# chjj/lcdb

Hardware: AMD Instinct MI355X
Metric: device-resident GiB/s Snappy encode+decode, 4 KiB blocks, 1/2/4/8 MI355X (higher is better)
Workload: dtype u8

## Files before the change

### lcdb_amd/csrc/lgs_api.cpp

```cpp

#include <hip/hip_runtime.h>

#include <stdarg.h>
#include <stdint.h>
#include <stdio.h>
#include <stdlib.h>
#include <string.h>
#include <unistd.h>

#include <atomic>
#include <chrono>
#include <condition_variable>
#include <deque>
#include <functional>
#include <memory>
#include <mutex>
#include <thread>
#include <unordered_map>
#include <vector>

#include "../../include/lcdb_gpu_snappy.h"

#include "lgs_block.h"
#include "lgs_launch.h"
// ... 748 lines not shown
      svc_stage(c, xp, n);
      uint32_t st = 0, olen = 0;
      const int rc = svc_call(*sv, c, 1, n, &st, &olen);
      if (rc == LGS_OK) {
        if (st == LGS_ST_OK && olen != want)
          return fail(LGS_EINTERNAL, "service decode: %u bytes for a %u-byte header", olen, want);
        if (st == LGS_ST_OK) memcpy(zp, h + kSvcOut, want);
        *ok = st == LGS_ST_OK;
        return LGS_OK;
      }
      if (rc != kSvcWithdrawn) return rc;
    }
  }

  Layout L;
  const size_t o_in = L.take((size_t)n + 16);
  const size_t o_ioff = L.take(8);
  const size_t o_ilen = L.take(4);
  const size_t o_ooff = L.take(8);
  const size_t o_ocap = L.take(4);
  const size_t up_end = L.at;
  const size_t o_st = L.take(4);
  const size_t o_olen = L.take(4);
  const size_t o_out = L.take((size_t)want + 16);
  const size_t down_end = L.at;
  if (down_end <= c.h_cap && want <= kInSlotDecodeMax) {
    uint8_t* const hd = c.h_dev;
    (void)up_end;
    memcpy(h + o_in, xp, n);
    memset(h + o_in + n, 0, 16);
    *(uint64_t*)(h + o_ioff) = o_in;
    *(uint32_t*)(h + o_ilen) = n;
    *(uint64_t*)(h + o_ooff) = o_out;
    *(uint32_t*)(h + o_ocap) = want;
    DecodeArgs a{hd, (const uint64_t*)(hd + o_ioff), (const uint32_t*)(hd + o_ilen), hd,
                 (const uint64_t*)(hd + o_ooff), (const uint32_t*)(hd + o_ocap),
                 (uint32_t*)(hd + o_olen), hd + o_st, nullptr, 1, nullptr};
    a.one = Item1{o_in, o_out, n, want, 1};
    LGS_HIP(launch_decode(a, want, c.stream));
    LGS_HIP(hipStreamSynchronize(c.stream));
    const uint8_t st = h[o_st];
    if (st == LGS_ST_OK) memcpy(zp, h + o_out, want);
    *ok = st == LGS_ST_OK;
    return LGS_OK;
  }
  std::unique_ptr<Scratch> guard;
  const size_t big_bytes = align_up((size_t)n + 16, 256) + align_up((size_t)want + 16, 256);
  LGS_TRY(big_alloc(&guard, big_bytes, want, c.stream));
  uint8_t* const big = (uint8_t*)guard->get();
  uint8_t* const d_in = big;
  uint8_t* const d_out = big + align_up((size_t)n + 16, 256);
  Layout M;
  const size_t m_ioff = M.take(8), m_ilen = M.take(4), m_ooff = M.take(8), m_ocap = M.take(4);
  const size_t m_up = M.at;
  const size_t m_st = M.take(4), m_olen = M.take(4);
  const size_t m_down = M.at;
  uint8_t* const d = c.d_buf;
  *(uint64_t*)(h + m_ioff) = 0;
  *(uint32_t*)(h + m_ilen) = n;
  *(uint64_t*)(h + m_ooff) = 0;
  *(uint32_t*)(h + m_ocap) = want;
  LGS_HIP(hipMemcpyAsync(d_in, xp, n, hipMemcpyHostToDevice, c.stream));
  LGS_HIP(hipMemsetAsync(d_in + n, 0, 16, c.stream));
  LGS_HIP(hipMemcpyAsync(d, h, m_up, hipMemcpyHostToDevice, c.stream));
  DecodeArgs a{d_in, (const uint64_t*)(d + m_ioff), (const uint32_t*)(d + m_ilen), d_out,
               (const uint64_t*)(d + m_ooff), (const uint32_t*)(d + m_ocap),
               (uint32_t*)(d + m_olen), d + m_st, nullptr, 1, nullptr};
  LGS_HIP(launch_decode(a, want, c.stream));
  LGS_HIP(hipMemcpyAsync(h + m_st, d + m_st, m_down - m_st, hipMemcpyDeviceToHost, c.stream));
  LGS_HIP(hipStreamSynchronize(c.stream));
  if (h[m_st] == LGS_ST_OK) {
    LGS_HIP(hipMemcpyAsync(zp, d_out, want, hipMemcpyDeviceToHost, c.stream));
    LGS_HIP(hipStreamSynchronize(c.stream));
    *ok = 1;
  }
  return LGS_OK;
}

Options& options_init() {
  static Options* o = [] {
    Options* v = new Options;
    const char* dk = getenv("LGS_DECODE_KERNEL");
    if (dk && !strcmp(dk, "ring")) v->decoder = kDecRing;
    if (dk && !strcmp(dk, "wave")) v->decoder = kDecWave;
#ifdef LGS_PROBE_DECODERS
    if (dk && !strcmp(dk, "chain")) v->decoder = kDecChain;
    if (dk && !strcmp(dk, "group")) v->decoder = kDecGroup;
    const char* wg = getenv("LGS_WIDE_DECODER");
    if (wg && !strcmp(wg, "group")) v->wide = kWideGroup;
    if (dk && !strcmp(dk, "quad")) v->decoder = kDecQuad;
    if (dk && !strcmp(dk, "ops")) v->decoder = kDecOps;
    const char* wd = getenv("LGS_WIDE_DECODER");
    if (wd && !strcmp(wd, "trips")) v->wide = kWideTrips;
#endif
#ifndef LGS_PROBE_DECODERS
    const char* wd0 = getenv("LGS_WIDE_DECODER");
    if ((dk && (!strcmp(dk, "quad") || !strcmp(dk, "ops") || !strcmp(dk, "group") ||
                !strcmp(dk, "chain"))) ||
        (wd0 && (!strcmp(wd0, "trips") || !strcmp(wd0, "group"))))
      fprintf(stderr,
              "lcdb_gpu_snappy: LGS_DECODE_KERNEL=%s LGS_WIDE_DECODER=%s names a probe-library "
              "decoder; this library uses its default decoders\n",
              dk ? dk : "", wd0 ? wd0 : "");
#endif
    const char* vo = getenv("LGS_VERIFY_OVERLAP");
    if (vo && !strcmp(vo, "0")) v->verify_overlap = 0;
    const char* ns = getenv("LGS_NO_SPLIT");
    if (ns && *ns && strcmp(ns, "0")) v->split = 0;
    return v;
  }();
  return *o;
}

}

int set_error(int code, const char* msg) { return fail(code, "%s", msg); }

Options& options() { return options_init(); }

hipError_t launch_fill_stride(uint64_t* off, uint64_t stride, uint32_t n, hipStream_t s);
hipError_t launch_check_lane(const CheckArgs& a, hipStream_t s);

}

using namespace lgs;

extern "C" {


int ldb_snappy_encode_size(size_t* zn, size_t xn) {
  if (xn > 0x7fffffff) return 0;
  const size_t n = bound_of(xn);
  if (n > 0x7fffffff) return 0;
  *zn = n;
  return 1;
}

size_t ldb_snappy_encode(uint8_t* zp, const uint8_t* xp, size_t xn) {
  size_t written = 0;
  if (encode_one(zp, xp, xn, &written) != LGS_OK) die("ldb_snappy_encode");
  return written;
}

int ldb_snappy_decode_size(size_t* zn, const uint8_t* xp, size_t xn) {
  uint32_t v;
  if (!read_varint32(&v, xp, xn)) return 0;
  if (v > 0x7fffffffu) return 0;
  *zn = v;
  return 1;
}

int ldb_snappy_decode(uint8_t* zp, const uint8_t* xp, size_t xn) {
  int ok = 0;
  if (decode_one(zp, xp, xn, &ok) != LGS_OK) die("ldb_snappy_decode");
  return ok;
}


int lgs_dropin_footprint(size_t* pinned, size_t* device, uint32_t* slots, size_t* slot_bytes) {
  if (!pinned || !device || !slots || !slot_bytes) return fail(LGS_EINVAL, "NULL argument");
  unsigned n = 0;
  dropin_pool().footprint(pinned, device, &n);
  *slots = n;
  *slot_bytes = dropin_pool().fixed_cap();
  return LGS_OK;
}

int lgs_service_quiesce(void) { return lgs::svc_quiesce(); }

int lgs_service_resume(void) {
  lgs::g_svc_paused = false;
  return LGS_OK;
}

int lgs_set_option(const char* name, const char* value) {
  if (!name || !value) return fail(LGS_EINVAL, "NULL argument");
  Options& o = options();
  if (!strcmp(name, "decoder")) {
    if (!strcmp(value, "auto") || !*value) o.decoder = kDecAuto;
    else if (!strcmp(value, "ring")) o.decoder = kDecRing;
    else if (!strcmp(value, "wave")) o.decoder = kDecWave;
#ifdef LGS_PROBE_DECODERS
    else if (!strcmp(value, "chain")) o.decoder = kDecChain;
    else if (!strcmp(value, "group")) o.decoder = kDecGroup;
    else if (!strcmp(value, "quad")) o.decoder = kDecQuad;
    else if (!strcmp(value, "ops")) o.decoder = kDecOps;
#endif
    else return fail(LGS_EINVAL, "decoder '%s' (auto, ring or wave)", value);
    return LGS_OK;
  }
  if (!strcmp(name, "inject_alloc_failures")) {
    char* end = nullptr;
    const long v = strtol(value, &end, 10);
    if (!*value || *end || v < 0 || v > 1000000)
      return fail(LGS_EINVAL, "inject_alloc_failures '%s' (0..1000000)", value);
    g_inject_alloc_failures = (int)v;
    return LGS_OK;
  }
  if (!strcmp(name, "wide")) {
    if (!strcmp(value, "walk") || !*value) o.wide = kWideWalk;
#ifdef LGS_PROBE_DECODERS
    else if (!strcmp(value, "group")) o.wide = kWideGroup;
    else if (!strcmp(value, "trips")) o.wide = kWideTrips;
#endif
    else return fail(LGS_EINVAL, "wide '%s' (walk)", value);
    return LGS_OK;
  }
  if (!strcmp(name, "service")) {
    if (!strcmp(value, "1")) g_svc_enabled = 1;
    else if (!strcmp(value, "0")) g_svc_enabled = 0;
    else return fail(LGS_EINVAL, "service '%s' (0 or 1)", value);
    return LGS_OK;
  }
  if (!strcmp(name, "verify_overlap")) {
    if (!strcmp(value, "1")) o.verify_overlap = 1;
    else if (!strcmp(value, "0")) o.verify_overlap = 0;
    else return fail(LGS_EINVAL, "verify_overlap '%s' (0 or 1)", value);
    return LGS_OK;
  }
  if (!strcmp(name, "split")) {
    if (!strcmp(value, "1")) o.split = 1;
    else if (!strcmp(value, "0")) o.split = 0;
    else return fail(LGS_EINVAL, "split '%s' (0 or 1)", value);
    return LGS_OK;
  }
  return fail(LGS_EINVAL, "unknown option '%s'", name);
}


size_t lgs_encode_bound(size_t n) { return bound_of(n); }

int lgs_encode_batch_dev(const uint8_t* d_in, const uint64_t* d_in_off, const uint32_t* d_in_len,
                         uint8_t* d_out, const uint64_t* d_out_off, uint32_t* d_out_len,
                         uint32_t n, uint32_t max_in_len, void* stream) {
  if (n == 0) return LGS_OK;
  if (!d_in || !d_in_off || !d_in_len || !d_out || !d_out_off || !d_out_len)
    return fail(LGS_EINVAL, "NULL argument");
  if (max_in_len > 0x7fffffffu) return fail(LGS_EINVAL, "max_in_len %u too large", max_in_len);
  EncodeArgs a{d_in, d_in_off, d_in_len, d_out, d_out_off, d_out_len, nullptr, nullptr, n, nullptr};
  LGS_HIP(launch_encode(a, max_in_len, (hipStream_t)stream));
  return LGS_OK;
}

int lgs_decode_batch_dev(const uint8_t* d_in, const uint64_t* d_in_off, const uint32_t* d_in_len,
                         uint8_t* d_out, const uint64_t* d_out_off, const uint32_t* d_out_cap,
                         uint32_t* d_out_len, uint8_t* d_status, uint32_t n,
                         uint32_t max_out_cap, void* stream) {
  if (n == 0) return LGS_OK;
  if (!d_in || !d_in_off || !d_in_len || !d_out || !d_out_off || !d_out_cap || !d_out_len ||
      !d_status)
    return fail(LGS_EINVAL, "NULL argument");
  DecodeArgs a{d_in, d_in_off, d_in_len, d_out, d_out_off, d_out_cap, d_out_len, d_status,
               nullptr, n, nullptr};
  LGS_HIP(launch_decode(a, max_out_cap, (hipStream_t)stream));
  return LGS_OK;
}

int lgs_encode_batch_host(const uint8_t* in, const uint64_t* in_off, const uint32_t* in_len,
                          uint8_t* out, const uint64_t* out_off, uint32_t* out_len, uint32_t n) {
  if (n == 0) return LGS_OK;
  if (!in || !in_off || !in_len || !out || !out_off || !out_len)
    return fail(LGS_EINVAL, "NULL argument");
  Lease lease(batch_pool());
// ... 1767 lines not shown
```

### lcdb_amd/csrc/lgs_decode.hip

```cpp
#include "lgs_device.h"
#include "lgs_decode_common.h"
#include "lgs_launch.h"
#include "lgs_probe_hooks.h"
#include "lgs_service.h"

#include <mutex>

namespace lgs {

__device__ uint32_t decode_win(const uint8_t* base, uint32_t sh, uint32_t slen, uint8_t* o,
                               int32_t gap, uint32_t cap, uint32_t* want_out) {
  const uint32_t lane = lane_id();

  const uint64_t w8 = uni64(lds_ld64(base, sh));
  uint32_t want = 0, hlen = 0;
  for (uint32_t i = 0; i < 5 && i < slen; ++i) {
    const uint32_t b = (uint32_t)(w8 >> (8 * i)) & 0xffu;
    if ((b & 0x80u) == 0) {
      want |= b << (7 * i);
      hlen = i + 1;
      break;
    }
    want |= (b & 0x7fu) << (7 * i);
  }
// ... 661 lines not shown
      const uint32_t j = __builtin_amdgcn_mbcnt_hi((uint32_t)(m >> 32),
                                                   __builtin_amdgcn_mbcnt_lo((uint32_t)m, 0));
      const uint32_t total = uni((uint32_t)__builtin_popcountll(m));
      if (need) {
        const uint64_t dp = reinterpret_cast<uint64_t>(dst);
        s_job[j] = RingJob(lane, F, fcnt, dp);
      }
      order();
#pragma clang loop unroll(disable)
      for (uint32_t base = 0; base < total; base += 16) {
        const uint32_t jj = base + (lane >> 2), w = lane & 3u;
        const RingJob jb = s_job[jj];
        if ((jj < total) & (16 * w < jb.cnt)) {
          const uint8_t* rb = s_out + (jb.lane() & (BL - 1)) * kOutStride + 16 +
                              ((uint32_t)jb.ptr() & 15u);
          const u32x4 v0 = lrd16(rb + ((jb.off + 16 * w) & (kOutRing - 1)));
          const bool two = 64 + 16 * w < jb.cnt;
          u32x4 v1 = v0;
          if (two) v1 = lrd16(rb + ((jb.off + 64 + 16 * w) & (kOutRing - 1)));
          const gptr<uint8_t> g = (gptr<uint8_t>)jb.ptr() + jb.off + 16 * w;
          LGS_RING_FLUSH_ST(g, v0, jb.cnt - 16 * w);
          if (two) LGS_RING_FLUSH_ST(g + 64, v1, jb.cnt - 64 - 16 * w);
        }
      }
      order();
      if (need) F += fcnt;
    }
    LGS_RING_PH(3);

    parse(false);
    LGS_RING_PH(4);
    if (TWO) {
      order();
      piece();
      order();
      parse(true);
    }
    LGS_RING_PH(5);

    {
      const uint32_t cons = ((orem > 0) & (okind == 0)) ? olp : pos;
      const bool need = (st == 1) & (in_req < slen) & (in_req <= cons + 64);
      const uint64_t m = ballot(need);
      const uint32_t j = __builtin_amdgcn_mbcnt_hi((uint32_t)(m >> 32),
                                                   __builtin_amdgcn_mbcnt_lo((uint32_t)m, 0));
      const uint32_t total = uni((uint32_t)__builtin_popcountll(m));
      if (need & (j < 32)) {
        const uint64_t sp = reinterpret_cast<uint64_t>(src);
        s_job[j] = RingJob(lane, in_req, slen, sp);
      }
      order();
      ra0 = rm0 = ra1 = rm1 = sink;
      const uint32_t w = lane & 3u;
      if ((lane >> 2) < total) {
        const RingJob jb = s_job[lane >> 2];
        const uint32_t o = jb.off + 16 * w;
        const gptr<const uint8_t> g = (gptr<const uint8_t>)jb.ptr();
        rv0 = ld16(g + (o < jb.cnt ? o : 0u));
        const uint32_t r = o & (kInRing - 1);
        ra0 = jb.lane() * kInStride + r;
        rm0 = r < 64 ? ra0 + kInRing : sink;
      }
      if (16 + (lane >> 2) < total) {
        const RingJob jb = s_job[16 + (lane >> 2)];
        const uint32_t o = jb.off + 16 * w;
        const gptr<const uint8_t> g = (gptr<const uint8_t>)jb.ptr();
        rv1 = ld16(g + (o < jb.cnt ? o : 0u));
        const uint32_t r = o & (kInRing - 1);
        ra1 = jb.lane() * kInStride + r;
        rm1 = r < 64 ? ra1 + kInRing : sink;
      }
      order();
      if (need & (j < 32)) in_req += 64;
    }
    LGS_RING_PH(6);
  } while (ballot(st == 1) & ~(ballot(orem == 0) & ballot(pos >= slen) & ballot(F >= made)));

  if (exists) {
    status[i] = (uint8_t)st;
    out_len[i] = LGS_RING_PH_VALUE(lane, LGS_RING_OUT_LEN(st == 1 ? want : 0));
  }
}

hipError_t launch_decode_ring(const DecodeArgs& a, hipStream_t s) {
#ifndef LGS_RING_BL
#define LGS_RING_BL 32
#endif
  hipLaunchKernelGGL((decode_ring_kernel<true, LGS_RING_BL>), dim3((a.n + LGS_RING_BL - 1) / LGS_RING_BL), dim3(64), 0, s, a.in,
                     a.in_off, a.in_len, a.out, a.out_off, a.out_cap, a.out_len, a.status,
                     a.index, a.n, a.count);
  return hipGetLastError();
}





constexpr uint32_t kDecCap0 = 4608;
constexpr uint32_t kDecCap1 = 16896;
constexpr uint32_t kDecCap2 = 66048;

constexpr uint32_t kLaneMinBlocks = 36864;

__global__ __launch_bounds__(256) void classify_kernel(const uint32_t* __restrict__ len,
                                                       uint32_t n, uint32_t b0, uint32_t b1,
                                                       uint32_t b2, uint32_t* __restrict__ list,
                                                       uint32_t* __restrict__ cnt) {
  const uint32_t i = blockIdx.x * 256 + threadIdx.x;
  const bool here = i < n;
  const uint32_t v = here ? len[i] : 0;
  const uint32_t c = v <= b0 ? 0 : v <= b1 ? 1 : v <= b2 ? 2 : 3;
  const uint32_t lane = lane_id();
  for (uint32_t k = 0; k < 4; ++k) {
    const uint64_t m = __ballot(here && c == k);
    if (m == 0) continue;
    const uint32_t leader = (uint32_t)__ffsll((unsigned long long)m) - 1;
    uint32_t base = 0;
    if (lane == leader) base = atomicAdd(&cnt[k], (uint32_t)__popcll(m));
    base = __shfl(base, leader);
    if (here && c == k) list[(size_t)k * n + base + __popcll(m & ((1ull << lane) - 1))] = i;
  }
}

hipError_t launch_classify(const uint32_t* len, uint32_t n, uint32_t b0, uint32_t b1, uint32_t b2,
                           uint32_t* list, uint32_t* cnt, hipStream_t s) {
  hipLaunchKernelGGL(classify_kernel, dim3((n + 255) / 256), dim3(256), 0, s, len, n, b0, b1, b2,
                     list, cnt);
  return hipGetLastError();
}

static hipMemPool_t scratch_pool(int dev, hipError_t* err) {
  static std::mutex mu;
  static hipMemPool_t pools[64] = {};
  std::lock_guard<std::mutex> g(mu);
  if (dev < 0 || dev >= 64) {
    *err = hipErrorInvalidDevice;
    return nullptr;
  }
  if (!pools[dev]) {
    hipMemPoolProps props = {};
    props.allocType = hipMemAllocationTypePinned;
    props.location.type = hipMemLocationTypeDevice;
    props.location.id = dev;
    hipMemPool_t p = nullptr;
    if ((*err = hipMemPoolCreate(&p, &props)) != hipSuccess) return nullptr;
    uint64_t keep = 256ull << 20;
    (void)hipMemPoolSetAttribute(p, hipMemPoolAttrReleaseThreshold, &keep);
    pools[dev] = p;
  }
  *err = hipSuccess;
  return pools[dev];
}

Scratch::Scratch(size_t bytes, hipStream_t s) : s_(s) {
  int dev = 0;
  err_ = hipGetDevice(&dev);
  if (err_ != hipSuccess) return;
  hipMemPool_t pool = scratch_pool(dev, &err_);
  if (err_ != hipSuccess) return;
  err_ = hipMallocFromPoolAsync(&p_, bytes, pool, s);
  if (err_ != hipSuccess) p_ = nullptr;
}

#define LGS_TRY(x) do { const hipError_t e_ = (x); if (e_ != hipSuccess) return e_; } while (0)

template <uint32_t OUT, uint32_t IN>
static hipError_t launch_decode_wide(const DecodeArgs& a, hipStream_t s) {
  hipLaunchKernelGGL((decode_wide_kernel<OUT, IN>), dim3(a.n), dim3(64), 0, s, a.in, a.in_off,
                     a.in_len, a.out, a.out_off, a.out_cap, a.out_len, a.status, a.index, a.n,
                     a.count);
  return hipGetLastError();
}
static hipError_t launch_decode_big(const DecodeArgs& a, uint32_t max_out, hipStream_t s) {
  (void)max_out;
#ifdef LGS_PROBE_DECODERS
  if (options().wide.load(std::memory_order_relaxed) == kWideTrips)
    return launch_decode_trips(a, s);
#endif
#ifdef LGS_PROBE_DECODERS
  if (max_out <= kGroupMaxOut && (options().wide.load(std::memory_order_relaxed) == kWideGroup ||
                                  options().decoder.load(std::memory_order_relaxed) == kDecGroup))
    return launch_decode_group(a, max_out, s);
#endif
  return launch_decode_wide<32768, 4096>(a, s);
}
static hipError_t launch_decode_mid(const DecodeArgs& a, hipStream_t s) {
  return launch_decode_cls<kDecCap1, 1>(a, s);
}

static hipError_t launch_decode_split(const DecodeArgs& a, uint32_t max_out, hipStream_t s) {
  const int force = options().decoder.load(std::memory_order_relaxed);
  const size_t list_bytes = (size_t)4 * a.n * sizeof(uint32_t);
  Scratch scratch(list_bytes + 16, s);
  LGS_TRY(scratch.status());
  uint32_t* list = (uint32_t*)scratch.get();
  uint32_t* cnt = (uint32_t*)((uint8_t*)scratch.get() + list_bytes);
  LGS_TRY(hipMemsetAsync(cnt, 0, 16, s));
  LGS_TRY(launch_classify(a.out_cap, a.n, kDecCap0, kDecCap1, kDecCap2, list, cnt, s));
  DecodeArgs c = a;
  c.index = list; c.count = cnt;
#ifdef LGS_PROBE_DECODERS
  if (options().decoder.load(std::memory_order_relaxed) == kDecOps) {
    LGS_TRY(launch_decode_ops(c, s));
  } else
#endif
  LGS_TRY((a.n >= kLaneMinBlocks || force == kDecRing ? launch_decode_ring(c, s)
                                                      : launch_decode_cls<kDecCap0, 1>(c, s)));
  c.index = list + a.n; c.count = cnt + 1;
  LGS_TRY(launch_decode_mid(c, s));
  if (max_out > kDecCap1) {
    c.index = list + 2 * (size_t)a.n; c.count = cnt + 2;
    LGS_TRY(launch_decode_big(c, kDecCap2, s));
  }
  if (max_out > kDecCap2) {
    c.index = list + 3 * (size_t)a.n; c.count = cnt + 3;
    LGS_TRY(launch_decode_big(c, max_out, s));
  }
  return scratch.release();
}

hipError_t launch_decode(const DecodeArgs& a, uint32_t max_out, hipStream_t s) {
  if (a.n == 0) return hipSuccess;
  if (a.one.on && (a.n != 1 || a.index)) return hipErrorInvalidValue;
  const int force = options().decoder.load(std::memory_order_relaxed);
#ifdef LGS_PROBE_DECODERS
  if (force == kDecOps && max_out <= kDecCap0) return launch_decode_ops(a, s);
  if (force == kDecQuad) return launch_decode_quad(a, s);
#endif
  if ((force == kDecAuto || force == kDecOps || force == kDecRing) &&
      !a.index && max_out > kDecCap0 && a.n >= kSplitMinBlocks &&
      options().split.load(std::memory_order_relaxed))
    return launch_decode_split(a, max_out, s);
  if (force == kDecRing || (force == kDecAuto && a.n >= kLaneMinBlocks))
    return launch_decode_ring(a, s);
#ifdef LGS_PROBE_DECODERS
  if (force == kDecGroup && max_out <= kGroupMaxOut) return launch_decode_group(a, max_out, s);
  if (force == kDecChain && max_out <= kChainMaxOut) return launch_decode_chain(a, max_out, s);
#endif
  if (max_out <= kDecCap0) return launch_decode_cls<kDecCap0, 1>(a, s);
  if (max_out <= kDecCap1) return launch_decode_mid(a, s);
  return launch_decode_big(a, max_out, s);
}

}
```

### lcdb_amd/csrc/lgs_launch.h

```cpp
#pragma once

#include <hip/hip_runtime.h>
#include <stddef.h>
#include <stdint.h>

#include <atomic>

namespace lgs {

enum DecodeKernel {
  kDecAuto = 0, kDecRing = 1, kDecWave = 2, kDecQuad = 3, kDecOps = 4, kDecGroup = 5, kDecChain = 6
};
enum WideKernel { kWideWalk = 0, kWideTrips = 1, kWideGroup = 2 };
struct Options {
  std::atomic<int> decoder{kDecAuto};
  std::atomic<int> split{1};
  std::atomic<int> wide{0};
  std::atomic<int> verify_overlap{1};
};
Options& options();

struct Item1 {
  uint64_t in_off = 0, out_off = 0;
  uint32_t in_len = 0, aux = 0;
  uint32_t on = 0;
};

struct DecodeArgs {
  const uint8_t* in; const uint64_t* in_off; const uint32_t* in_len;
  uint8_t* out; const uint64_t* out_off; const uint32_t* out_cap;
  uint32_t* out_len; uint8_t* status; const uint32_t* index; uint32_t n;
  const uint32_t* count;
  Item1 one{};
};

struct EncodeArgs {
  const uint8_t* in; const uint64_t* in_off; const uint32_t* in_len;
  uint8_t* out; const uint64_t* out_off; uint32_t* out_len;
  const uint32_t* hdr; const uint32_t* index; uint32_t n;
  const uint32_t* count;
  Item1 one{};
};

hipError_t launch_decode(const DecodeArgs& a, uint32_t max_out, hipStream_t s);
#ifdef LGS_PROBE_DECODERS
hipError_t launch_decode_quad(const DecodeArgs& a, hipStream_t s);
hipError_t launch_decode_ops(const DecodeArgs& a, hipStream_t s);
hipError_t launch_decode_trips(const DecodeArgs& a, hipStream_t s);
#endif
hipError_t launch_decode_ring(const DecodeArgs& a, hipStream_t s);

#ifdef LGS_PROBE_DECODERS
constexpr uint32_t kGroupMaxOut = 66048;
hipError_t launch_decode_group(const DecodeArgs& a, uint32_t max_out, hipStream_t s);
constexpr uint32_t kChainMaxOut = 16896;
hipError_t launch_decode_chain(const DecodeArgs& a, uint32_t max_out, hipStream_t s);
#endif
hipError_t launch_encode(const EncodeArgs& a, uint32_t max_in, hipStream_t s);
constexpr uint32_t kSplitMinBlocks = 512;
hipError_t launch_classify(const uint32_t* len, uint32_t n, uint32_t b0, uint32_t b1, uint32_t b2,
                           uint32_t* list, uint32_t* cnt, hipStream_t s);
class Scratch {
 public:
  Scratch(size_t bytes, hipStream_t s);
  ~Scratch() { (void)release(); }
  Scratch(const Scratch&) = delete;
  Scratch& operator=(const Scratch&) = delete;
  hipError_t status() const { return err_; }
  void* get() const { return p_; }
  hipError_t release() {
    void* p = p_;
    p_ = nullptr;
    return p ? hipFreeAsync(p, s_) : hipSuccess;
  }

 private:
  void* p_ = nullptr;
  hipStream_t s_;
  hipError_t err_;
};

constexpr uint32_t kSvcMaxSlots = 64;
constexpr uint32_t kSvcMaxItem = 4608;
constexpr uint32_t kSvcIn = 0;
constexpr uint32_t kSvcOut = 8192;

struct alignas(128) SvcMailbox {
  uint32_t req;
  uint32_t len;
  uint32_t aux;
  uint32_t stop;
  uint64_t arena;
  uint64_t pad0[5];
  uint32_t ack;
// ... 79 lines not shown
```

### lcdb_amd/csrc/lgs_probe_hooks.h

```cpp
#pragma once

#include <stdint.h>

#ifdef LGS_PROBE_RING_PHASES
#define LGS_RING_PH_DECL                                   \
  uint32_t ph_[8] = {0, 0, 0, 0, 0, 0, 0, 0};               \
  uint32_t ph_trips_ = 0;                                   \
  uint64_t ph_t_ = __builtin_amdgcn_s_memtime()
#define LGS_RING_PH(k)                                     \
  do {                                                     \
    const uint64_t t_ = __builtin_amdgcn_s_memtime();      \
    ph_[k] += (uint32_t)(t_ - ph_t_);                      \
    ph_t_ = t_;                                            \
  } while (0)
#define LGS_RING_PH_TRIP() (++ph_trips_)
#define LGS_RING_PH_VALUE(lane, dflt) lgs_ring_ph_value_(ph_, ph_trips_, (lane), (dflt))
#define LGS_RING_PH_ACTIVE 1
__device__ __forceinline__ uint32_t lgs_ring_ph_value_(const uint32_t* ph, uint32_t trips,
                                                       uint32_t lane, uint32_t dflt) {
  uint32_t v = lane == 8 ? trips : dflt;
#pragma unroll
  for (uint32_t k = 0; k < 8; ++k) v = lane == k ? ph[k] : v;
  return v;
}
#else
#define LGS_RING_PH_DECL do {} while (0)
#define LGS_RING_PH(k) do {} while (0)
#define LGS_RING_PH_TRIP() do {} while (0)
#define LGS_RING_PH_VALUE(lane, dflt) (dflt)
#define LGS_RING_PH_ACTIVE 0
#endif

#ifdef LGS_PROBE_TRIPCOUNT
#define LGS_RING_TRIPS_DECL uint32_t trips_ = 0
#define LGS_RING_TRIP() (++trips_)
#define LGS_RING_OUT_LEN(v) (trips_)
#else
#define LGS_RING_TRIPS_DECL do {} while (0)
#define LGS_RING_TRIP() do {} while (0)
#define LGS_RING_OUT_LEN(v) (v)
#endif

#ifdef LGS_PROBE_NOFAR
#define LGS_RING_FAR_LD16(p) ((void)(p), u32x4{0, 0, 0, 0})
#else
#define LGS_RING_FAR_LD16(p) ld16(p)
#endif
#ifdef LGS_PROBE_NOFLUSH
#define LGS_RING_FLUSH_ST(g, v, c) \
  do { if ((v).x == 0x12345678u && (c) == 77777u) st16((g), (v)); } while (0)
#else
#define LGS_RING_FLUSH_ST(g, v, c) \
  do { if ((c) >= 16) st16((g), (v)); else st_exact((g), (v), (c)); } while (0)
#endif

#ifdef LGS_PROBE_DEC_TIMING
#define LGS_DEC_PH_DECL                                                   \
  const uint64_t dtp0_ = __builtin_amdgcn_s_memtime();                    \
  const uint64_t drt0_ = __builtin_amdgcn_s_memrealtime();                \
  uint64_t dtp1_ = dtp0_
#define LGS_DEC_PH_STAGED()                                               \
  do { __builtin_amdgcn_s_waitcnt(0); dtp1_ = __builtin_amdgcn_s_memtime(); } while (0)
#define LGS_DEC_PH_END(FLUSH_STMT, STORE_PTR)                             \
  do {                                                                    \
    __builtin_amdgcn_s_waitcnt(0);                                        \
    const uint64_t tp2_ = __builtin_amdgcn_s_memtime();                   \
    FLUSH_STMT;                                                           \
    __builtin_amdgcn_s_waitcnt(0);                                        \
    const uint64_t tp3_ = __builtin_amdgcn_s_memtime();                   \
    const uint64_t rt3_ = __builtin_amdgcn_s_memrealtime();               \
    if (lane_id() == 0) {                                                 \
      gptr<uint32_t> q_ = (STORE_PTR);                                    \
      q_[0] = (uint32_t)(dtp1_ - dtp0_);                                  \
      q_[1] = (uint32_t)(tp2_ - dtp1_);                                   \
      q_[2] = (uint32_t)(tp3_ - tp2_);                                    \
      q_[3] = (uint32_t)(rt3_ - drt0_);                                   \
    }                                                                     \
  } while (0)
#else
#define LGS_DEC_PH_DECL do {} while (0)
#define LGS_DEC_PH_STAGED() do {} while (0)
#define LGS_DEC_PH_END(FLUSH_STMT, STORE_PTR) do {} while (0)
#endif

#ifdef LGS_PROBE_FORCE_REPLAY
#define LGS_ENC_REPLAY(cond, vmask) (vmask)
#else
#define LGS_ENC_REPLAY(cond, vmask) (ballot(cond) & (vmask))
#endif
#ifdef LGS_PROBE_ENC_TIMING
#define LGS_ENC_PH_DECL                                                   \
  const uint64_t etp0_ = __builtin_amdgcn_s_memtime();                    \
  uint64_t etp1_ = etp0_
#define LGS_ENC_PH_STAGED()                                               \
  do { __builtin_amdgcn_s_waitcnt(0); etp1_ = __builtin_amdgcn_s_memtime(); } while (0)
#define LGS_ENC_PH_END(SLOT, LEN)                                         \
  do {                                                                    \
    __builtin_amdgcn_s_waitcnt(0);                                        \
    const uint64_t tp2_ = __builtin_amdgcn_s_memtime();                   \
    if (lane_id() == 0) {                                                 \
      const uint32_t b_ = 32 + (LEN) + (LEN) / 6 - 16;                    \
      (SLOT).put4(0, b_, (uint32_t)(etp1_ - etp0_));                      \
      (SLOT).put4(0, b_ + 4, (uint32_t)(tp2_ - etp1_));                   \
      (SLOT).put4(0, b_ + 8, 0x7e57u);                                    \
    }                                                                     \
  } while (0)
#else
#define LGS_ENC_PH_DECL do {} while (0)
#define LGS_ENC_PH_STAGED() do {} while (0)
#define LGS_ENC_PH_END(SLOT, LEN) do {} while (0)
#endif
```

Before: 319.1.

## Add two-wave walker/mover pair decoder as default ring decode path

Introduces decode_pair_kernel, in which one wavefront parses Snappy tags and refills the input ring while a second wavefront consumes a shared LDS queue of pieces and performs copies and flushes to global memory. The two wavefronts hand off through double-buffered barriers. The intent is to overlap tag parsing with data movement, which the single-wave ring kernel does serially. The old ring kernel stays reachable as 'ring32', and the auto threshold for choosing the ring path is lowered, so more batches take the new kernel. The cost is added barrier synchronisation and higher LDS use per block.

```diff
diff --git a/lcdb_amd/csrc/lgs_api.cpp b/lcdb_amd/csrc/lgs_api.cpp
--- a/lcdb_amd/csrc/lgs_api.cpp
+++ b/lcdb_amd/csrc/lgs_api.cpp
@@ -854,6 +854,7 @@
     Options* v = new Options;
     const char* dk = getenv("LGS_DECODE_KERNEL");
     if (dk && !strcmp(dk, "ring")) v->decoder = kDecRing;
+    if (dk && !strcmp(dk, "ring32")) v->decoder = kDecRing32;
     if (dk && !strcmp(dk, "wave")) v->decoder = kDecWave;
 #ifdef LGS_PROBE_DECODERS
     if (dk && !strcmp(dk, "chain")) v->decoder = kDecChain;
@@ -951,6 +952,7 @@
   if (!strcmp(name, "decoder")) {
     if (!strcmp(value, "auto") || !*value) o.decoder = kDecAuto;
     else if (!strcmp(value, "ring")) o.decoder = kDecRing;
+    else if (!strcmp(value, "ring32")) o.decoder = kDecRing32;
     else if (!strcmp(value, "wave")) o.decoder = kDecWave;
 #ifdef LGS_PROBE_DECODERS
     else if (!strcmp(value, "chain")) o.decoder = kDecChain;
diff --git a/lcdb_amd/csrc/lgs_decode.hip b/lcdb_amd/csrc/lgs_decode.hip
--- a/lcdb_amd/csrc/lgs_decode.hip
+++ b/lcdb_amd/csrc/lgs_decode.hip
@@ -767,7 +767,388 @@
   }
 }
 
+namespace pairq {
+constexpr uint32_t kBlocks = 64, kDepth = 8, kRefillJobs = 32;
+constexpr uint32_t kCopy = 0x40u;
+constexpr uint32_t kMaxOut = 0xffffffu;
+constexpr uint32_t kRej = 0x8000u, kFin = 0x4000u;
+constexpr uint32_t kIn = 192, kNone = 0xffffffffu;
+static_assert(kIn + 16 == ring::kInStride, "the input ring and its mirror fill ring::kInStride");
+__device__ __forceinline__ uint32_t in_at(uint32_t pos) {
+  return pos - kIn * (__umulhi(pos, 0xAAAAAAABu) >> 7);
+}
+constexpr uint32_t kLdsBytes =
+    kBlocks * (ring::kInStride + ring::kOutStride) + (kBlocks + kRefillJobs) * 16 +
+    kDepth * kBlocks * 4 + 2 * kBlocks * 2 + 2 * kBlocks + 2 * 4;
+static_assert(kLdsBytes <= 40960, "decode_pair_kernel: more than a quarter of a CU's LDS");
+}
+
+__device__ __forceinline__ void pair_barrier() {
+  asm volatile("s_waitcnt lgkmcnt(0)\n\ts_barrier" ::: "memory");
+}
+
+__device__ __forceinline__ void pair_piece(uint8_t* ob, const uint8_t* ib, uint32_t lo, bool lit,
+                                           uint32_t dist, uint32_t piece, uint32_t made) {
+  using namespace ring;
+  const bool overlap = !lit & (dist < piece);
+  const bool pat = overlap & (dist <= 8) & ((dist & (dist - 1)) == 0);
+  if (overlap & !pat) {
+    const uint32_t qq = dist >= 16 ? dist : dist * ((16 + dist - 1) / dist);
+    u32x4 p0;
+    if (dist >= 16) {
+      p0 = lrd16(ob + ((made - dist) & (kOutRing - 1)));
+    } else {
+      const u32x4 c0 = lrd16(ob + ((made - dist) & (kOutRing - 1)));
+      uint32_t w[4] = {0, 0, 0, 0};
+      uint32_t r = 0;
+#pragma clang loop unroll(disable)
+      for (uint32_t j = 0; j < 16; ++j) {
+        w[j >> 2] |= byte_of(c0, r) << (8 * (j & 3u));
+        r = r + 1 == dist ? 0 : r + 1;
+      }
+      p0 = u32x4{w[0], w[1], w[2], w[3]};
+    }
+    out_put(ob, made, p0);
+    order();
+#pragma clang loop unroll(disable)
+    for (uint32_t k = 1; 16 * k < piece; ++k) {
+      const u32x4 v = lrd16(ob + ((made + 16 * k - qq) & (kOutRing - 1)));
+      out_put(ob, made + 16 * k, v);
+      order();
+    }
+  } else {
+    const uint8_t* const cp = ob + ((made - dist) & (kOutRing - 1));
+    auto src = [&](uint32_t k) {
+      const uint32_t o = lo + 16 * k;
+      return lit ? ib + (o >= pairq::kIn ? o - pairq::kIn : o) : cp + 16 * k;
+    };
+    const u32x4 c0 = lrd16(src(0));
+    const uint32_t w1 = __builtin_amdgcn_perm(c0.x, c0.x, 0x00000000u);
+    const uint32_t w2 = __builtin_amdgcn_perm(c0.x, c0.x, 0x01000100u);
+    const uint32_t px = dist == 1 ? w1 : (dist == 2 ? w2 : c0.x);
+    const uint32_t py = dist == 8 ? c0.y : px;
+    const u32x4 pv = {px, py, px, py};
+    out_put(ob, made, pat ? pv : c0);
+    if (piece > 16) out_put(ob, made + 16, pat ? pv : lrd16(src(1)));
+    if (piece > 32) out_put(ob, made + 32, pat ? pv : lrd16(src(2)));
+    if (piece > 48) out_put(ob, made + 48, pat ? pv : lrd16(src(3)));
+  }
+}
+
+__global__ __launch_bounds__(128) void decode_pair_kernel(
+    const uint8_t* __restrict__ in, const uint64_t* __restrict__ in_off,
+    const uint32_t* __restrict__ in_len, uint8_t* __restrict__ out,
+    const uint64_t* __restrict__ out_off, const uint32_t* __restrict__ out_cap,
+    uint32_t* __restrict__ out_len, uint8_t* __restrict__ status,
+    const uint32_t* __restrict__ index, uint32_t n,
+    const uint32_t* __restrict__ count) {
+  using namespace ring;
+  using namespace pairq;
+  __shared__ __attribute__((aligned(16))) uint8_t s_in[kBlocks * kInStride];
+  __shared__ __attribute__((aligned(16))) uint8_t s_out[kBlocks * kOutStride];
+  __shared__ __attribute__((aligned(16))) RingJob s_fjob[kBlocks];
+  __shared__ __attribute__((aligned(16))) RingJob s_rjob[kRefillJobs];
+  __shared__ uint32_t s_q[kDepth][kBlocks];
+  __shared__ uint16_t s_qtail[2][kBlocks];
+  __shared__ uint8_t s_qdone[2][kBlocks];
+  __shared__ uint32_t s_exit[2];
+  static_assert(sizeof(s_in) + sizeof(s_out) + sizeof(s_fjob) + sizeof(s_rjob) + sizeof(s_q) +
+                    sizeof(s_qtail) + sizeof(s_qdone) + sizeof(s_exit) == kLdsBytes,
+                "decode_pair_kernel: LDS layout and kLdsBytes disagree");
+
+  const uint32_t lane = threadIdx.x & 63u;
+  const bool walker = uni(threadIdx.x >> 6) == 0;
+  const uint32_t slot = blockIdx.x * kBlocks + lane;
+  if (count) n = *count;
+  if (blockIdx.x * kBlocks >= n) return;
+  const bool exists = slot < n;
+  const uint32_t i = exists ? (index ? index[slot] : slot) : 0;
+  const gptr<const uint8_t> src = to_global(in) + (exists ? in_off[i] : 0);
+  const uint32_t slen = exists ? in_len[i] : 0;
+  const gptr<uint8_t> dst = to_global(out) + (exists ? out_off[i] : 0);
+  const uint32_t cap = exists ? out_cap[i] : 0;
+
+  uint32_t st = exists ? 1u : 3u, want = 0, hlen = 0;
+  if (exists) {
+    const uint64_t h = view8(src);
+    for (uint32_t k = 0; k < 5 && k < slen; ++k) {
+      const uint32_t b = (uint32_t)(h >> (8 * k)) & 0xffu;
+      if ((b & 0x80u) == 0) {
+        want |= b << (7 * k);
+        hlen = k + 1;
+        break;
+      }
+      want |= (b & 0x7fu) << (7 * k);
+    }
+    if (hlen == 0 || want > 0x7fffffffu) st = 0;
+    else if ((want > cap) | (want > kMaxOut)) st = 2;
+  }
+  __builtin_amdgcn_s_waitcnt(0x0f70);
+  LGS_PAIR_PH_DECL;
+
+  if (walker) {
+    uint8_t* const ib = s_in + lane * kInStride;
+    uint32_t pos = hlen;
+    uint32_t wmade = 0;
+    uint32_t in_req = 0, in_have = 0;
+    uint32_t in_req_at = 0;
+    uint32_t wrem = 0, wx = 0, wlow = hlen;
+    bool wlit = false;
+    uint32_t qtail = 0;
+    uint32_t lw0 = 0, lw1 = 0, lw2 = 0, lw3 = 0, lw4 = 0, lw5 = 0, lw6 = 0, lw7 = 0;
+    u32x4 rv0 = {0, 0, 0, 0}, rv1 = rv0;
+    uint32_t ra0 = kNone, rm0 = kNone, ra1 = kNone, rm1 = kNone;
+
+    auto slot_step = [&](uint32_t qd) {
+      const uint32_t need_to = slen - pos < 5 ? slen : pos + 5;
+      const bool ready = (st == 1) & (wrem == 0) & (pos < slen) & (in_have >= need_to);
+      const Tag t = parse_tag(rrd_tag(ib + in_at(pos)), pos, slen, want, wmade);
+      if (ready & t.bad) st = 0;
+      const bool take = ready & !t.bad;
+      wrem = take ? t.len : wrem;
+      wlit = take ? t.kind == 0 : wlit;
+      wx = take ? (t.kind == 0 ? pos + t.hl : t.dist) : wx;
+      wlow = take ? (t.kind == 0 ? pos + t.hl : t.next) : wlow;
+      wmade += take ? t.len : 0u;
+      pos = take ? t.next : pos;
+
+      const uint32_t plen = wrem < 64 ? wrem : 64;
+      const bool room = ((qtail - qd) & 0xffu) < kDepth;
+      if ((st == 1) & (wrem > 0) & room & (!wlit | (in_have >= wx + plen))) {
+        const uint32_t k = qtail & (kDepth - 1);
+        s_q[k][lane] = (plen - 1) | (wlit ? in_at(wx) << 8 : kCopy | wx << 8);
+        lw0 = k == 0 ? wlow : lw0;
+        lw1 = k == 1 ? wlow : lw1;
+        lw2 = k == 2 ? wlow : lw2;
+        lw3 = k == 3 ? wlow : lw3;
+        lw4 = k == 4 ? wlow : lw4;
+        lw5 = k == 5 ? wlow : lw5;
+        lw6 = k == 6 ? wlow : lw6;
+        lw7 = k == 7 ? wlow : lw7;
+        ++qtail;
+        wrem -= plen;
+        if (wlit) {
+          wx += plen;
+          wlow = wx;
+        }
+      }
+    };
+
+    s_qtail[1][lane] = 0;
+    pair_barrier();
+    uint32_t par = 0, go;
+    do {
+      LGS_PAIR_PH_TRIP();
+      LGS_PAIR_PH(7);
+      const uint32_t qd = s_qdone[par ^ 1][lane];
+
+      __builtin_amdgcn_s_waitcnt(0x0f70);
+      LGS_PAIR_PH(0);
+      if (ra0 != kNone) lwr16(s_in + ra0, rv0);
+      if (rm0 != kNone) lwr16(s_in + rm0, rv0);
+      if (ra1 != kNone) lwr16(s_in + ra1, rv1);
+      if (rm1 != kNone) lwr16(s_in + rm1, rv1);
+      order();
+      in_have = in_req;
+      LGS_PAIR_PH(1);
+
+      slot_step(qd);
+      order();
+      LGS_PAIR_PH(2);
+      slot_step(qd);
+      order();
+      LGS_PAIR_PH(3);
+
+      const bool ended = (st == 1) & (wrem == 0) & (pos >= slen);
+      if (ended & (wmade != want)) st = 0;
+      s_qtail[par][lane] = (uint16_t)((qtail & 0xffu) | (st == 0 ? kRej : 0u) |
+                                      ((ended & (st == 1)) ? kFin : 0u));
+
+      {
+        const uint32_t k = qd & (kDepth - 1);
+        const uint32_t lwa = k == 0 ? lw0 : (k == 1 ? lw1 : (k == 2 ? lw2 : lw3));
+        const uint32_t lwb = k == 4 ? lw4 : (k == 5 ? lw5 : (k == 6 ? lw6 : lw7));
+        const uint32_t lwq = k < 4 ? lwa : lwb;
+        const uint32_t cons = ((qtail - qd) & 0xffu) != 0 ? lwq : (wrem > 0 ? wlow : pos);
+        const bool need = (st == 1) & (in_req < slen) & (in_req <= cons + (kIn - 64));
+        const uint64_t m = ballot(need);
+        const uint32_t j = __builtin_amdgcn_mbcnt_hi((uint32_t)(m >> 32),
+                                                     __builtin_amdgcn_mbcnt_lo((uint32_t)m, 0));
+        const uint32_t total = uni((uint32_t)__builtin_popcountll(m));
+        if (need & (j < kRefillJobs)) {
+          const uint64_t sp = reinterpret_cast<uint64_t>(src);
+          s_rjob[j] = RingJob(lane, in_req_at, slen - in_req, sp + in_req);
+        }
+        order();
+        ra0 = rm0 = ra1 = rm1 = kNone;
+        const uint32_t w = lane & 3u;
+        if ((lane >> 2) < total) {
+          const RingJob jb = s_rjob[lane >> 2];
+          const gptr<const uint8_t> g = (gptr<const uint8_t>)jb.ptr();
+          rv0 = ld16(g + (16 * w < jb.cnt ? 16 * w : 0u));
+          const uint32_t r = jb.off + 16 * w;
+          ra0 = jb.lane() * kInStride + r;
+          rm0 = r == 0 ? ra0 + kIn : kNone;
+        }
+        if (16 + (lane >> 2) < total) {
+          const RingJob jb = s_rjob[16 + (lane >> 2)];
+          const gptr<const uint8_t> g = (gptr<const uint8_t>)jb.ptr();
+          rv1 = ld16(g + (16 * w < jb.cnt ? 16 * w : 0u));
+          const uint32_t r = jb.off + 16 * w;
+          ra1 = jb.lane() * kInStride + r;
+          rm1 = r == 0 ? ra1 + kIn : kNone;
+        }
+        order();
+        if (need & (j < kRefillJobs)) {
+          in_req += 64;
+          in_req_at = in_req_at == kIn - 64 ? 0u : in_req_at + 64;
+        }
+      }
+      LGS_PAIR_PH(4);
+
+      pair_barrier();
+      go = uni(s_exit[par]);
+      par ^= 1;
+    } while (go);
+    LGS_PAIR_PH_END_WALKER(exists, lane, out_len + i);
+    return;
+  }
+
+  uint8_t* const ob = s_out + lane * kOutStride + 16 +
+                      ((uint32_t)reinterpret_cast<uintptr_t>(dst) & 15u);
+  const uint8_t* const ib = s_in + lane * kInStride;
+  uint32_t made = 0, F = 0;
+  uint32_t qhead = 0;
+  bool have = false, ofar = false, olit = false;
+  uint32_t olen = 0, ox = 0;
+  u32x4 fa0 = {0, 0, 0, 0}, fa1 = fa0, fa2 = fa0, fa3 = fa0;
+
+  auto slot_step = [&](uint32_t e, uint32_t tail, bool second) {
+    const uint32_t len = (e & 63u) + 1, x = e >> 8;
+    const bool lit = (e & kCopy) == 0;
+    const bool far = !lit & (x > kNear);
+    const bool take = (st == 1) & !have & (((tail - qhead) & 0xffu) != 0) &
+                      (!second | !far | (made - F + len <= x));
+    if (take) {
+      have = true;
+      olen = len;
+      ox = x;
+      olit = lit;
+      ofar = far;
+      ++qhead;
+      if (far) {
+        const gptr<const uint8_t> sp = (gptr<const uint8_t>)(dst + (made - x));
+        fa0 = LGS_RING_FAR_LD16(sp);
+        if (len > 16) {
+          fa1 = LGS_RING_FAR_LD16(sp + 16);
+          if (len > 32) {
+            fa2 = LGS_RING_FAR_LD16(sp + 32);
+            if (len > 48) fa3 = LGS_RING_FAR_LD16(sp + 48);
+          }
+        }
+      }
+    }
+    if ((st == 1) & have & !ofar) {
+      pair_piece(ob, ib, ox, olit, ox, olen, made);
+      made += olen;
+      have = false;
+    }
+  };
+
+  s_qdone[1][lane] = 0;
+  pair_barrier();
+  uint32_t par = 0;
+  uint64_t live;
+  do {
+    LGS_PAIR_PH_TRIP();
+    LGS_PAIR_PH(7);
+    const uint32_t pub = s_qtail[par ^ 1][lane];
+    const uint32_t e0 = s_q[qhead & (kDepth - 1)][lane];
+    const uint32_t e1 = s_q[(qhead + 1) & (kDepth - 1)][lane];
+
+    __builtin_amdgcn_s_waitcnt(0x0f70);
+    LGS_PAIR_PH(0);
+    if ((st == 1) & have) {
+      out_put(ob, made, fa0);
+      if (olen > 16) out_put(ob, made + 16, fa1);
+      if (olen > 32) out_put(ob, made + 32, fa2);
+      if (olen > 48) out_put(ob, made + 48, fa3);
+      made += olen;
+      have = false;
+    }
+    order();
+    if ((st == 1) & ((pub & kRej) != 0)) st = 0;
+    LGS_PAIR_PH(1);
+
+    const bool fin = (st == 1) & ((pub & kFin) != 0) & (((pub - qhead) & 0xffu) == 0);
+    const uint64_t dpa = reinterpret_cast<uint64_t>(dst);
+    const uint64_t lb = (dpa + made) & ~(uint64_t)(kFlush - 1);
+    const uint32_t lim = lb > dpa ? (uint32_t)(lb - dpa) : 0u;
+    const uint32_t fcnt = lim > F ? lim - F : (fin ? made - F : 0u);
+    {
+      const bool need = (st == 1) & (fcnt > 0);
+      const uint64_t m = ballot(need);
+      const uint32_t j = __builtin_amdgcn_mbcnt_hi((uint32_t)(m >> 32),
+                                                   __builtin_amdgcn_mbcnt_lo((uint32_t)m, 0));
+      const uint32_t total = uni((uint32_t)__builtin_popcountll(m));
+      if (need) s_fjob[j] = RingJob(lane, F, fcnt, dpa);
+      order();
+      constexpr uint32_t kFL = 2, kFG = 8 / kFL;
+#pragma clang loop unroll(disable)
+      for (uint32_t base = 0; base < total; base += 64 / kFL) {
+        const uint32_t jj = base + lane / kFL, w = lane % kFL;
+        const RingJob jb = s_fjob[jj];
+        if ((jj < total) & (16 * w < jb.cnt)) {
+          const uint8_t* rb = s_out + (jb.lane() & (kBlocks - 1)) * kOutStride + 16 +
+                              ((uint32_t)jb.ptr() & 15u);
+          const gptr<uint8_t> g = (gptr<uint8_t>)jb.ptr() + jb.off;
+          u32x4 v[kFG];
+#pragma unroll
+          for (uint32_t k = 0; k < kFG; ++k) {
+            const uint32_t o = 16 * (w + kFL * k);
+            if (k > 0) v[k] = v[0];
+            if (k == 0 || o < jb.cnt) v[k] = lrd16(rb + ((jb.off + o) & (kOutRing - 1)));
+          }
+#pragma unroll
+          for (uint32_t k = 0; k < kFG; ++k) {
+            const uint32_t o = 16 * (w + kFL * k);
+            if (o < jb.cnt) LGS_RING_FLUSH_ST(g + o, v[k], jb.cnt - o);
+          }
+        }
+      }
+      order();
+      if (need) F += fcnt;
+    }
+    LGS_PAIR_PH(2);
+
+    slot_step(e0, pub, false);
+    order();
+    LGS_PAIR_PH(3);
+    slot_step(e1, pub, true);
+    order();
+    LGS_PAIR_PH(4);
+
+    s_qdone[par][lane] = (uint8_t)(qhead - (have ? 1u : 0u));
+    live = ballot((st == 1) & !(fin & (F >= made)));
+    if (lane == 0) s_exit[par] = live != 0;
+    pair_barrier();
+    par ^= 1;
+  } while (live != 0);
+
+  if (exists) {
+    status[i] = (uint8_t)st;
+    out_len[i] = st == 1 ? want : 0;
+  }
+  LGS_PAIR_PH_END_MOVER(exists, lane, out_len + i);
+}
+
 hipError_t launch_decode_ring(const DecodeArgs& a, hipStream_t s) {
+  if (options().decoder.load(std::memory_order_relaxed) != kDecRing32) {
+    hipLaunchKernelGGL(decode_pair_kernel, dim3((a.n + pairq::kBlocks - 1) / pairq::kBlocks),
+                       dim3(128), 0, s, a.in, a.in_off, a.in_len, a.out, a.out_off, a.out_cap,
+                       a.out_len, a.status, a.index, a.n, a.count);
+    return hipGetLastError();
+  }
 #ifndef LGS_RING_BL
 #define LGS_RING_BL 32
 #endif
@@ -785,7 +1166,7 @@
 constexpr uint32_t kDecCap1 = 16896;
 constexpr uint32_t kDecCap2 = 66048;
 
-constexpr uint32_t kLaneMinBlocks = 36864;
+constexpr uint32_t kLaneMinBlocks = 28672;
 
 __global__ __launch_bounds__(256) void classify_kernel(const uint32_t* __restrict__ len,
                                                        uint32_t n, uint32_t b0, uint32_t b1,
@@ -874,7 +1255,8 @@
 }
 
 static hipError_t launch_decode_split(const DecodeArgs& a, uint32_t max_out, hipStream_t s) {
-  const int force = options().decoder.load(std::memory_order_relaxed);
+  int force = options().decoder.load(std::memory_order_relaxed);
+  if (force == kDecRing32) force = kDecRing;
   const size_t list_bytes = (size_t)4 * a.n * sizeof(uint32_t);
   Scratch scratch(list_bytes + 16, s);
   LGS_TRY(scratch.status());
@@ -907,7 +1289,9 @@
 hipError_t launch_decode(const DecodeArgs& a, uint32_t max_out, hipStream_t s) {
   if (a.n == 0) return hipSuccess;
   if (a.one.on && (a.n != 1 || a.index)) return hipErrorInvalidValue;
-  const int force = options().decoder.load(std::memory_order_relaxed);
+  int force = options().decoder.load(std::memory_order_relaxed);
+  const bool ring32 = force == kDecRing32;
+  if (ring32) force = kDecRing;
 #ifdef LGS_PROBE_DECODERS
   if (force == kDecOps && max_out <= kDecCap0) return launch_decode_ops(a, s);
   if (force == kDecQuad) return launch_decode_quad(a, s);
@@ -916,7 +1300,8 @@
       !a.index && max_out > kDecCap0 && a.n >= kSplitMinBlocks &&
       options().split.load(std::memory_order_relaxed))
     return launch_decode_split(a, max_out, s);
-  if (force == kDecRing || (force == kDecAuto && a.n >= kLaneMinBlocks))
+  if ((force == kDecRing || (force == kDecAuto && a.n >= kLaneMinBlocks)) &&
+      (ring32 || max_out <= pairq::kMaxOut))
     return launch_decode_ring(a, s);
 #ifdef LGS_PROBE_DECODERS
   if (force == kDecGroup && max_out <= kGroupMaxOut) return launch_decode_group(a, max_out, s);
diff --git a/lcdb_amd/csrc/lgs_launch.h b/lcdb_amd/csrc/lgs_launch.h
--- a/lcdb_amd/csrc/lgs_launch.h
+++ b/lcdb_amd/csrc/lgs_launch.h
@@ -9,7 +9,8 @@
 namespace lgs {
 
 enum DecodeKernel {
-  kDecAuto = 0, kDecRing = 1, kDecWave = 2, kDecQuad = 3, kDecOps = 4, kDecGroup = 5, kDecChain = 6
+  kDecAuto = 0, kDecRing = 1, kDecWave = 2, kDecQuad = 3, kDecOps = 4, kDecGroup = 5, kDecChain = 6,
+  kDecRing32 = 7
 };
 enum WideKernel { kWideWalk = 0, kWideTrips = 1, kWideGroup = 2 };
 struct Options {
diff --git a/lcdb_amd/csrc/lgs_probe_hooks.h b/lcdb_amd/csrc/lgs_probe_hooks.h
--- a/lcdb_amd/csrc/lgs_probe_hooks.h
+++ b/lcdb_amd/csrc/lgs_probe_hooks.h
@@ -29,6 +29,30 @@
 #define LGS_RING_PH_TRIP() do {} while (0)
 #define LGS_RING_PH_VALUE(lane, dflt) (dflt)
 #define LGS_RING_PH_ACTIVE 0
+#endif
+
+#ifdef LGS_PROBE_RING_PHASES
+#define LGS_PAIR_PH_DECL LGS_RING_PH_DECL
+#define LGS_PAIR_PH(k) LGS_RING_PH(k)
+#define LGS_PAIR_PH_TRIP() LGS_RING_PH_TRIP()
+#define LGS_PAIR_PH_END_MOVER(ok, lane, ptr)                              \
+  do {                                                                    \
+    if ((ok) && (lane) <= 8) *(ptr) = lgs_ring_ph_value_(ph_, ph_trips_, (lane), 0u); \
+    __builtin_amdgcn_s_waitcnt(0x0f70);                                   \
+    pair_barrier();                                                       \
+  } while (0)
+#define LGS_PAIR_PH_END_WALKER(ok, lane, ptr)                             \
+  do {                                                                    \
+    pair_barrier();                                                       \
+    if ((ok) && (lane) >= 16 && (lane) <= 24)                             \
+      *(ptr) = lgs_ring_ph_value_(ph_, ph_trips_, (lane) - 16, 0u);       \
+  } while (0)
+#else
+#define LGS_PAIR_PH_DECL do {} while (0)
+#define LGS_PAIR_PH(k) do {} while (0)
+#define LGS_PAIR_PH_TRIP() do {} while (0)
+#define LGS_PAIR_PH_END_MOVER(ok, lane, ptr) do {} while (0)
+#define LGS_PAIR_PH_END_WALKER(ok, lane, ptr) do {} while (0)
 #endif
 
 #ifdef LGS_PROBE_TRIPCOUNT
```

New measurement: 327.8 (median of 6 runs). +2.7%, better.
